# suleka96/siddhi

Hardware: AMD Instinct MI355X
Metric: input events/sec + % HBM peak, partitioned pattern query, 1/2/4/8 MI355X (higher is better)
Workload: dtype f64

## Files before the change

### siddhi_amd/csrc/kernels/fastpath.h

```cpp
#pragma once
#include "nfa.h"
#include "primitives.h"
#include "stream_ops.h"

namespace sm {

struct FastArgs {
  int64_t n;
  const int64_t* ts;
  const NfaStream* st;
  const KeyProg* key;
  const Instr* code;
  const DVal* consts;
  int c1_off, c1_len, c2_off, c2_len;
  int64_t within;
  const int64_t* ordinals;
  int64_t ordinal_base;
};

struct FastHostInfo {
  const void* const* cols;
  const int32_t* types;
  int key_col = -1;
  int key_type = 0;
// ... 43 lines not shown
    ts_last = 0;
  }
};

int64_t fast_every_within(const FastArgs& a, uint32_t* pairs_out, int64_t pairs_cap, Scratch& sc, hipStream_t s,
                          FastTimings* tm = nullptr);

enum : int64_t { FAST_OUTSIDE = -1, FAST_NON_MONOTONE = -2, FAST_KEY_SPAN = -3 };

int64_t fast_every_within_v2(const FastArgs& a, const FastHostInfo& hi, FastState& fs, FastCarry& carry,
                             uint32_t* pairs_out, int64_t pairs_cap, Scratch& sc, hipStream_t s,
                             FastTimings* tm = nullptr, int stack_mode = 0);

int64_t fast_seq_adjacent(const FastArgs& a, const FastHostInfo& hi, FastState& fs, FastCarry& carry,
                          uint32_t* pairs_out, int64_t pairs_cap, Scratch& sc, hipStream_t s, FastTimings* tm = nullptr);


struct StackPlan {
  const void* rec;
  const uint32_t* dbase;
  int64_t n;
  int64_t omax;
  int H;
  int64_t kmin;
  int op;
  bool fp;
  bool exact_codes;
  int vtype, vattr, vmode;
  int64_t vmin;
  const void* vcol;
  int64_t within;
  int64_t ts0, ts_last;
  int32_t o0;
};

int64_t stack_pipeline(const StackPlan& p, const FastArgs& a, const FastHostInfo& hi, FastState& fs, FastCarry& carry,
                       uint32_t* pairs_out, int64_t pairs_cap, Scratch& sc, hipStream_t s, FastTimings* tm);

void build_carry(const int64_t* cand, int64_t ncand, const NfaStream* st, int nattr, FastCarry& carry, Scratch& sc,
                 hipStream_t s, int key_bits = 64, int64_t kmin = 0, bool key_runs_ordered = false);

void pair_project(const uint32_t* pairs, int64_t m, const NfaStream* st_dev, const int64_t* ord, int64_t n,
                  int64_t base, const int64_t* ts, const int64_t* prev_carry, int64_t nc, int cw, const char* blob_dev,
                  DVal* out, int64_t* ts_out, Scratch& sc, hipStream_t s, bool rows = false,
                  int64_t* words = nullptr, uint8_t* nulls = nullptr,
                  const uint32_t* carry_keys = nullptr, const uint32_t* carry_idx = nullptr, bool sync = true);
void pair_project_carry_order(const int64_t* prev_carry, int64_t nc, int cw, int64_t base, Scratch& sc, hipStream_t s,
                              const uint32_t** carry_keys, const uint32_t** carry_idx);

}
```

### siddhi_amd/csrc/kernels/fastpath3.hip

```cpp
#include <cstdlib>
#include <type_traits>
#include <vector>

#include "expr.h"
#include "fastpath.h"
#include "fastpath_dev.h"
#include "pass0_dev.h"

#ifndef SM_ORIG_NT_LOAD
#define SM_ORIG_NT_LOAD 1
#endif

namespace sm {

namespace {

#ifndef SM_SB
#define SM_SB 512
#endif
#ifndef SM_SI
#define SM_SI 8
#endif
constexpr int kBlock = SM_SB;
constexpr int kWaves = kBlock / 64;
constexpr int kItems = SM_SI;
constexpr int kTile = kBlock * kItems;
constexpr int kBinsPerThread = kBins >= kBlock ? kBins / kBlock : 1;
constexpr int kUpUnroll = 8;
#ifndef SM_WB
#define SM_WB 512
#endif
#ifndef SM_WI
#define SM_WI 4
// ... 141 lines not shown
    unsigned long long e = __shfl_down(vlo, o, 64), f = __shfl_down(vhi, o, 64);
    lo = x < lo ? x : lo;
    hi = y > hi ? y : hi;
    om = z > om ? z : om;
    vlo = e < vlo ? e : vlo;
    vhi = f > vhi ? f : vhi;
  }
  bad = __any(bad) ? 1u : 0u;
  bado = __any(bado) ? 1u : 0u;
  if (lane == 0) {
    if (kcol) {
      atomicMin(&c->kmin, lo);
      atomicMax(&c->kmax, hi);
    }
    if (vlong) {
      atomicMin(&c->vmin, vlo);
      atomicMax(&c->vmax, vhi);
    }
    if (ord) atomicMax(&c->omax, om);
    if (bad) atomicOr(&c->bad_ts, 1u);
    if (bado) atomicOr(&c->bad_ord, 1u);
  }
  if (blockIdx.x == 0 && threadIdx.x == 0) {
    c->ts0 = ts[0];
    c->ts_last = ts[n - 1];
    c->o0 = ord ? ord[0] - obase : 0;
    if (!ord) c->omax = (unsigned long long)(n - 1);
  }
  __syncthreads();
  if (kcol)
    for (int d = threadIdx.x; d < kBins; d += kBlock) cnt[(int64_t)d * G + blockIdx.x] = h[d];
}


template <typename KT>
struct KeyColDigits {
  const KT* kcol;
  int64_t kmin;
  __device__ uint32_t key(int64_t p) const { return (uint32_t)((int64_t)kcol[p] - kmin); }
};
struct RecDigits {
  const uint4* r;
  __device__ uint32_t key(int64_t p) const { return ((const uint32_t*)r)[4 * p]; }
};
struct PairDigits {
  const uint64_t* q;
  __device__ uint32_t key(int64_t p) const { return (uint32_t)(q[p] >> 32); }
};

template <typename DS>
__global__ void __launch_bounds__(kBlock) upsweep_kernel(DS src, int64_t n, int64_t per, int G, int shift,
                                                         uint32_t* __restrict__ cnt) {
  __shared__ uint32_t h[kBins];
  for (int d = threadIdx.x; d < kBins; d += kBlock) h[d] = 0;
  __syncthreads();
  int64_t lo, len;
  chunk_range(blockIdx.x, n, per, nullptr, lo, len);
  const int64_t hi = lo + len;
  for (int64_t b = lo; b < hi; b += (int64_t)kBlock * kUpUnroll) {
    uint32_t k[kUpUnroll];
#pragma unroll
    for (int u = 0; u < kUpUnroll; ++u) {
      const int64_t p = b + u * kBlock + threadIdx.x;
      k[u] = p < hi ? src.key(p) : 0u;
    }
#pragma unroll
// ... 33 lines not shown
  uint32_t v[kBinsPerThread], s = 0;
  for (int k = 0; k < kBinsPerThread; ++k) {
    const int d = threadIdx.x * kBinsPerThread + k;
    v[k] = d < kBins ? tot[d] : 0u;
    s += v[k];
  }
  const int lane = threadIdx.x & 63, w = threadIdx.x >> 6;
  const uint32_t inc = wave_incl_scan(s);
  if (lane == 63) lw[w] = inc;
  __syncthreads();
  uint32_t run = inc - s;
  for (int k = 0; k < w; ++k) run += lw[k];
  for (int k = 0; k < kBinsPerThread; ++k) {
    if (threadIdx.x * kBinsPerThread + k < kBins) tot[threadIdx.x * kBinsPerThread + k] = run;
    run += v[k];
  }
}


template <typename VT>
struct ValLoader {
  VT v;
  __device__ StackVal var(const Instr&) const {
    StackVal r;
    r.i = 0;
    r.d = 0;
    r.null = 0;
    if constexpr (std::is_floating_point<VT>::value) r.d = (double)v;
    else r.i = (int64_t)v;
    return r;
  }
};

template <typename KT, typename VT>
struct OrigSrc {
  const NfaStream* st;
  const KT* kcol;
  const VT* vcol;
  int64_t kmin;
  int vmode;
  int64_t vmin;
  const uint64_t* c1mask;
  const int64_t* ts;
  int64_t ts0;
  const int64_t* ord;
  int64_t obase;
  const Instr* c1code;
  int c1len;
  const DVal* consts;
  bool c1_inline;
  Cond c1;
  __device__ void init() {
    if (c1_inline) c1 = make_cond(c1code, c1len, consts);
  }
  __device__ uint32_t c1_bit(VT v, uint64_t m, int64_t p) const {
    if (c1_inline) return eval_simple(c1, ValLoader<VT>{v}) ? 1u : 0u;
    return (uint32_t)(m >> (p & 63)) & 1u;
  }
  __device__ uint4 rec(int64_t p) const {
    uint4 r;
    const VT v = vcol[p];
    const uint64_t m = c1_inline ? 0ull : c1mask[p >> 6];
    r.x = (uint32_t)((int64_t)kcol[p] - kmin) | (c1_bit(v, m, p) << 31);
    r.y = ord ? (uint32_t)(ord[p] - obase) : (uint32_t)p;
    r.z = vcode<VT>(v, vmode, vmin);
    r.w = (uint32_t)(ts[p] - ts0);
    return r;
  }
  struct Raw {
    uint32_t k;
    VT v;
    uint32_t t, o, m;
  };
  __device__ Raw load(int64_t p) const {
    Raw r;
    const uint32_t* t32 = (const uint32_t*)(ts + p);
#if SM_ORIG_NT_LOAD
    r.k = __builtin_nontemporal_load((const uint32_t*)(kcol + p));
    r.v = __builtin_nontemporal_load(vcol + p);
    r.t = __builtin_nontemporal_load(t32);
    if (ord) r.o = __builtin_nontemporal_load((const uint32_t*)(ord + p));
#else
    r.k = *(const uint32_t*)(kcol + p);
    r.v = vcol[p];
    r.t = *t32;
    if (ord) r.o = *(const uint32_t*)(ord + p);
#endif
    if (!c1_inline) r.m = ((const uint32_t*)c1mask)[p >> 5];
    return r;
  }
  __device__ uint32_t rel_ord(const Raw& r, int64_t p) const { return ord ? r.o - (uint32_t)obase : (uint32_t)p; }
  __device__ uint32_t c1_of(const Raw& r, int64_t p) const {
    if (c1_inline) return eval_simple(c1, ValLoader<VT>{r.v}) ? 1u : 0u;
    return (r.m >> (p & 31)) & 1u;
  }
  __device__ void split(const Raw& r, int64_t p, uint64_t& a, uint64_t& b) const {
    const uint32_t c1 = c1_of(r, p);
    a = (uint64_t)((r.k - (uint32_t)kmin) | (c1 << 31)) | ((uint64_t)rel_ord(r, p) << 32);
    b = (uint64_t)vcode<VT>(r.v, vmode, vmin) | ((uint64_t)(r.t - (uint32_t)ts0) << 32);
  }
  __device__ uint4 record(const Raw& r, int64_t p) const {
    const uint32_t c1 = c1_of(r, p);
    return make_uint4((r.k - (uint32_t)kmin) | (c1 << 31), rel_ord(r, p), vcode<VT>(r.v, vmode, vmin),
                      r.t - (uint32_t)ts0);
  }
  __device__ void flush() {}
};

struct RecSrc {
  const uint4* r;
  __device__ void init() {}
  typedef unsigned int Raw __attribute__((ext_vector_type(4)));
  __device__ uint4 rec(int64_t p) const {
    const Raw v = __builtin_nontemporal_load((const Raw*)r + p);
    return make_uint4(v.x, v.y, v.z, v.w);
  }
  __device__ Raw load(int64_t p) const { return __builtin_nontemporal_load((const Raw*)r + p); }
  __device__ void split(const Raw& v, int64_t, uint64_t& a, uint64_t& b) const {
    a = (uint64_t)v.x | ((uint64_t)v.y << 32);
    b = (uint64_t)v.z | ((uint64_t)v.w << 32);
  }
};

struct PairSrc {
  const uint64_t* q;
  __device__ void init() {}
  using Raw = uint64_t;
  __device__ Raw load(int64_t p) const { return __builtin_nontemporal_load(q + p); }
  __device__ void split(const Raw& v, int64_t, uint64_t& a, uint64_t&) const { a = v; }
};

template <int MODE, typename Src>
__global__ void __launch_bounds__(kBlock) __attribute__((amdgpu_waves_per_eu(4)))
downsweep_kernel(Src src, uint4* __restrict__ drec, uint64_t* __restrict__ dpairs, int64_t n, int64_t per,
                 const uint32_t* seg_len, int G, int shift, const uint32_t* __restrict__ cnt,
                 const uint32_t* __restrict__ dbase) {
  __shared__ uint64_t xb64[kTile];
// ... 972 lines not shown

bool sort_wc() {
  static const bool on = [] {
    const char* e = getenv("SM_SORT_WC");
    return !(e && e[0] == '0');
  }();
  return on;
}

int jpass_wc() {
  static const int v = [] {
    const char* e = getenv("SM_JPASS_WC");
    return e ? atoi(e) : 0;
  }();
  return v;
}

bool c1_inline(const FastHostInfo& hi, const FastArgs& a) {
  if (!hi.c1_host || hi.c1_len != a.c1_len) return false;
  if (hi.c1_len != 0) {
    const Instr* c = hi.c1_host;
    auto leaf = [](const Instr& in) { return in.op != OP_CMP && in.op != OP_MATH && in.op != OP_NOT; };
    if (hi.c1_len != 3 || c[2].op != OP_CMP || !leaf(c[0]) || !leaf(c[1])) return false;
  }
  for (int k = 0; k < hi.c1_len; ++k) {
    const Instr& in = hi.c1_host[k];
    if (in.op == OP_TS) return false;
    if (in.op == OP_VAR && (in.a != 0 || in.c != hi.vattr)) return false;
    if (in.op == OP_COL && in.a != hi.vattr) return false;
  }
  return true;
}

template <typename KT, typename VT>
void launch_down0_t(const FastHostInfo& hi, const FastArgs& a, const void* kcol, int64_t kmin, int vmode, int64_t vmin,
                    const uint64_t* c1mask, int64_t ts0, int G, int64_t per, hipStream_t s, uint4* dst,
                    const uint32_t* cnt, const uint32_t* dbase) {
  OrigSrc<KT, VT> os{a.st, (const KT*)kcol, (const VT*)hi.cols[hi.vattr], kmin, vmode, vmin, c1mask, a.ts, ts0,
                     a.ordinals, a.ordinal_base, a.code + a.c1_off, a.c1_len, a.consts, c1_inline(hi, a)};
  static const bool p0v2 = !(getenv("SM_PASS0_V2") && getenv("SM_PASS0_V2")[0] == '0');
  if (sort_wc() && p0v2)
    hipLaunchKernelGGL((pass0_kernel<OrigSrc<KT, VT>>), dim3(G), dim3(kP0Block), 0, s, os, dst, a.n, per, G, cnt, dbase);
  else if (sort_wc())
    hipLaunchKernelGGL((downsweep_wc_kernel<0, OrigSrc<KT, VT>>), dim3(G), dim3(kWcBlock), 0, s, os, dst, nullptr, a.n,
                       per, nullptr, G, 0, cnt, dbase);
  else
    hipLaunchKernelGGL((downsweep_kernel<0, OrigSrc<KT, VT>>), dim3(G), dim3(kBlock), 0, s, os, dst, nullptr, a.n, per,
                       nullptr, G, 0, cnt, dbase);
}

template <typename KT>
void launch_down0_k(const FastHostInfo& hi, const FastArgs& a, const void* kcol, int64_t kmin, int vmode, int64_t vmin,
                    const uint64_t* m, int64_t ts0, int G, int64_t per, hipStream_t s, uint4* dst,
                    const uint32_t* cnt, const uint32_t* dbase) {
  switch (hi.vtype) {
    case T_INT: launch_down0_t<KT, int32_t>(hi, a, kcol, kmin, vmode, vmin, m, ts0, G, per, s, dst, cnt, dbase); break;
    case T_LONG: launch_down0_t<KT, int64_t>(hi, a, kcol, kmin, vmode, vmin, m, ts0, G, per, s, dst, cnt, dbase); break;
    case T_FLOAT: launch_down0_t<KT, float>(hi, a, kcol, kmin, vmode, vmin, m, ts0, G, per, s, dst, cnt, dbase); break;
    case T_DOUBLE: launch_down0_t<KT, double>(hi, a, kcol, kmin, vmode, vmin, m, ts0, G, per, s, dst, cnt, dbase); break;
    default: throw std::runtime_error("fast path: unsupported compared-attribute type");
  }
}

int64_t round_up(int64_t x, int64_t m) { return (x + m - 1) / m * m; }


struct ResolveArgs {
  const int64_t* crow;
  int64_t nc;
  int w, vattr, vtype, vmode;
  int64_t vmin;
  bool exact_codes;
  const uint4* rec;
  const NfaStream* st;
  const int64_t* ts;
  const int64_t* ord;
  int64_t obase, n, kmin, span, ts0, within;
  uint64_t* cpair;
  int64_t* cand;
  uint32_t* cand_n;
  uint32_t cand_cap;
  uint32_t* err;
};

template <bool KEYED, int OP, bool FP>
__global__ void resolve_kernel(ResolveArgs r) {
  const int64_t i = (int64_t)blockIdx.x * blockDim.x + threadIdx.x;
  if (i >= r.nc) return;
  const int64_t* row = r.crow + i * r.w;
  const int64_t key = row[0], oc = row[1], tc = row[2];
  const StackVal vc = uncanon((uint64_t)row[3 + r.vattr], r.vtype);
  r.cpair[i] = ~0ull;
// ... 183 lines not shown

  if (fs.cus == 0) {
    int dev = 0;
    SM_HIP(hipGetDevice(&dev));
    SM_HIP(hipDeviceGetAttribute(&fs.cus, hipDeviceAttributeMultiprocessorCount, dev));
  }
  if (fs.sort_wgs_per_cu == 0) {
    int b = 0;
    if (sort_wc()) SM_HIP(hipOccupancyMaxActiveBlocksPerMultiprocessor(&b, downsweep_wc_kernel<1, RecSrc>, kWcBlock, 0));
    else SM_HIP(hipOccupancyMaxActiveBlocksPerMultiprocessor(&b, downsweep_kernel<1, RecSrc>, kBlock, 0));
    fs.sort_wgs_per_cu = std::max(1, b);
    b = 0;
    SM_HIP(hipOccupancyMaxActiveBlocksPerMultiprocessor(&b, walk_kernel<true, CMP_GT, true>, kWalkBlock, 0));
    fs.walk_wgs_per_cu = std::max(1, b);
  }
  constexpr int kOversub = 2;
  const int64_t tiles = (n + kTile - 1) / kTile;
  const int G = (int)std::max<int64_t>(1, std::min<int64_t>(tiles, (int64_t)kOversub * fs.sort_wgs_per_cu * fs.cus));
  const int64_t per = round_up((n + G - 1) / G, kTile);
  const int64_t wtiles = (n + kWalkTile - 1) / kWalkTile;
  const int Gw = (int)std::max<int64_t>(1, std::min<int64_t>(wtiles, (int64_t)fs.walk_wgs_per_cu * fs.cus));
  const int64_t perw = round_up((n + Gw - 1) / Gw, kWalkTile);
  uint32_t* cnt = (uint32_t*)sc.take(sizeof(uint32_t) * kBins * std::max(G, Gw));
  uint32_t* dbase = (uint32_t*)sc.take(sizeof(uint32_t) * kBins);
  uint32_t* mcount = (uint32_t*)sc.take(sizeof(uint32_t) * Gw);
  uint64_t* c1mask = (uint64_t*)sc.take(((n + 63) / 64) * 8);
  auto scan_counts = [&](int g) {
    hipLaunchKernelGGL(scan_chunks_kernel, dim3(kBins), dim3(256), 0, s, cnt, g, dbase);
    hipLaunchKernelGGL(digit_base_kernel, dim3(1), dim3(kBlock), 0, s, dbase);
    tmark("scan");
  };

  const bool mask = !keyed || !c1_inline(hi, a);
#define SM_PREP2(KT, M, X)                                                                                          \
  hipLaunchKernelGGL((prep_kernel<KT, M, X>), dim3(G), dim3(kBlock), 0, s, (const KT*)kcol, vlong, a.ts, a.ordinals, \
                     a.ordinal_base, n, per, G, a.st, a.code + a.c1_off, a.c1_len, a.consts, c1mask, cnt, c)
#define SM_PREP(KT, M)                  \
  do {                                  \
    if (a.ordinals || vlong)            \
      SM_PREP2(KT, M, true);            \
    else                                \
      SM_PREP2(KT, M, false);           \
  } while (0)
  if (key_type == T_LONG && keyed) {
    if (mask) SM_PREP(int64_t, true);
    else SM_PREP(int64_t, false);
  } else {
    if (mask) SM_PREP(int32_t, true);
    else SM_PREP(int32_t, false);
  }
#undef SM_PREP
#undef SM_PREP2
  tmark("prep");
  Ctrl hc;
  SM_HIP(hipMemcpyAsync(&hc, c, sizeof(Ctrl), hipMemcpyDeviceToHost, s));
  SM_HIP(hipStreamSynchronize(s));
  if (a.within >= 0) {
    if (hc.bad_ts || (carry.active && hc.ts0 < carry.ts_last)) {
      sc.used = mark;
      return FAST_NON_MONOTONE;
    }
    if ((unsigned long long)(hc.ts_last - hc.ts0) >= 0xffffffffull) return bail();
  }
  if (hc.omax >= 0x7fffffffull || hc.bad_ord) return bail();
  int kbits = 0;
  int64_t kmin = 0;
  uint64_t kspan = 0;
  if (keyed) {
    kmin = (int64_t)(hc.kmin ^ 0x8000000000000000ull);
    kmin &= ~(int64_t)(kBins - 1);
    kspan = (uint64_t)((int64_t)(hc.kmax ^ 0x8000000000000000ull) - kmin);
    kbits = std::max(1, bits_for(kspan));
    if (kbits > 30 || (hi.remap_span > 0 && kspan > (uint64_t)hi.remap_span)) {
      sc.used = mark;
      return FAST_KEY_SPAN;
    }
  }
  int vmode = VC_I32;
  int64_t vmin = 0;
  bool exact_codes = true;
  switch (hi.vtype) {
    case T_INT: vmode = VC_I32; break;
    case T_FLOAT: vmode = VC_F32; break;
    case T_DOUBLE: vmode = VC_F64; exact_codes = false; break;
    default:
      if (keyed && carry.n == 0 && hc.vmax - hc.vmin <= 0xffffffffull) {
        vmode = VC_I64R;
        vmin = (int64_t)(hc.vmin ^ 0x8000000000000000ull);
      } else {
        vmode = VC_I64H;
        exact_codes = false;
      }
  }
  const int fpass = keyed ? (kbits + kRB - 1) / kRB : 0;
  const int jbits = std::max(1, bits_for(hc.omax));
  const int jpass = (jbits + kRB - 1) / kRB;
  auto finish = [&](int64_t m) {
    carry.ts_last = carry.active ? std::max<int64_t>(carry.ts_last, hc.ts_last) : (int64_t)hc.ts_last;
    carry.active = true;
    sc.used = mark;
    return m;
  };

  uint64_t* stq = nullptr;
  uint64_t *pq = nullptr, *qq = nullptr;
  WalkArgs wa{};
  wa.st = a.st;
  wa.ts = a.ts;
  wa.ord = a.ordinals;
  wa.obase = a.ordinal_base;
  wa.c1 = a.code + a.c1_off;
  wa.c1_len = a.c1_len;
  wa.c2 = a.code + a.c2_off;
  wa.c2_len = a.c2_len;
  wa.consts = a.consts;
  wa.vattr = hi.vattr;
  wa.vtype = hi.vtype;
  wa.within = a.within;
  wa.n = n;
  wa.exact_codes = exact_codes;
  wa.c1mask = c1mask;
  wa.kmin = kmin;
  wa.ts0 = hc.ts0;
  const int64_t nc = carry.n;
  const int64_t cand_cap = std::min<int64_t>(n + nc, (int64_t)1 << 26) + 1024;
  uint32_t* cflags = (uint32_t*)sc.take(16);
  SM_HIP(hipMemsetAsync(cflags, 0, 16, s));
  int64_t* cand = nullptr;
  uint4* cur = nullptr;
  if (keyed) {
    uint4* A = (uint4*)sc.take(n * 16);
    uint4* B = (uint4*)sc.take(n * 16);
    scan_counts(G);
    if (key_type == T_INT)
      launch_down0_k<int32_t>(hi, a, kcol, kmin, vmode, vmin, c1mask, hc.ts0, G, per, s, A, cnt, dbase);
    else launch_down0_k<int64_t>(hi, a, kcol, kmin, vmode, vmin, c1mask, hc.ts0, G, per, s, A, cnt, dbase);
    tmark("key_pass0");
    const int H = (int)std::min<uint64_t>(kspan >> kRB, 1ull << 20) + 1;
    const bool order_op = spec >= 0 && (spec >> 1) != CMP_EQ && (spec >> 1) != CMP_NE;
    const bool ts_ok = a.within < 0 || (a.within < (1ll << 30) && hc.ts_last - hc.ts0 < (1ll << 30));
    if (stack_mode != 2 && order_op && ts_ok && H <= kBins && (stack_mode == 1 || H >= kBins / 2)) {
      StackPlan sp{};
      sp.rec = A;
      sp.dbase = dbase;
      sp.n = n;
      sp.omax = (int64_t)hc.omax;
      sp.H = H;
      sp.kmin = kmin;
      sp.op = spec >> 1;
      sp.fp = (spec & 1) != 0;
      sp.exact_codes = exact_codes;
      sp.vtype = hi.vtype;
      sp.vattr = hi.vattr;
      sp.vmode = vmode;
      sp.vmin = vmin;
      sp.vcol = hi.cols[hi.vattr];
      sp.within = a.within;
      sp.ts0 = hc.ts0;
      sp.ts_last = hc.ts_last;
      sp.o0 = (int32_t)hc.o0;
      const int64_t m = stack_pipeline(sp, a, hi, fs, carry, pairs_out, pairs_cap, sc, s, tm);
      if (m >= 0) {
        fs.last_path = 3;
        if (tm) {
          SM_HIP(hipEventRecord(tm->ev[1], s));
          SM_HIP(hipEventRecord(tm->ev[2], s));
          SM_HIP(hipEventRecord(tm->ev[3], s));
        }
        return finish(m);
      }
    }
    cand = (int64_t*)sc.take((size_t)cand_cap * 32);
    cur = A;
    uint4* nxt = B;
    for (int p = 1; p < fpass; ++p) {
      hipLaunchKernelGGL((upsweep_kernel<RecDigits>), dim3(G), dim3(kBlock), 0, s, RecDigits{cur}, n, per, G,
                         p * kRB, cnt);
      tmark("key_up");
      scan_counts(G);
      if (sort_wc())
        hipLaunchKernelGGL((downsweep_wc_kernel<1, RecSrc>), dim3(G), dim3(kWcBlock), 0, s, RecSrc{cur}, nxt, nullptr, n,
                           per, nullptr, G, p * kRB, cnt, dbase);
      else
        hipLaunchKernelGGL((downsweep_kernel<1, RecSrc>), dim3(G), dim3(kBlock), 0, s, RecSrc{cur}, nxt, nullptr, n,
                           per, nullptr, G, p * kRB, cnt, dbase);
      tmark("key_pass");
      std::swap(cur, nxt);
    }
    if (tm) SM_HIP(hipEventRecord(tm->ev[1], s));
    wa.rec = cur;
    wa.cand = cand;
    wa.cand_n = cflags;
    wa.cand_cap = (uint32_t)cand_cap;
    wa.err = cflags + 1;
// ... 162 lines not shown
```

### siddhi_amd/csrc/kernels/pass0_dev.h

```cpp
#pragma once
#include "fastpath_dev.h"

namespace sm {
namespace {

constexpr int kP0Block = 1024;
constexpr int kP0Waves = kP0Block / 64;
constexpr int kP0Items = 4;
constexpr int kP0Tile = kP0Block * kP0Items;
constexpr int kP0Seg = 4;
static_assert(kBins == kP0Block && kP0Waves == 16, "one digit per thread, 16 waves");

__device__ __forceinline__ uint32_t sm_udot2(uint32_t a, uint32_t b, uint32_t c) {
#if defined(__HIP_DEVICE_COMPILE__)
  typedef unsigned short u16x2 __attribute__((ext_vector_type(2)));
  return __builtin_amdgcn_udot2(__builtin_bit_cast(u16x2, a), __builtin_bit_cast(u16x2, b), c, false);
#else
  return c + (a & 0xffffu) * (b & 0xffffu) + (a >> 16) * (b >> 16);
#endif
}

__device__ __forceinline__ uint32_t p0_before(const uint4& r0, const uint4& r1, int w) {
  const uint32_t word[8] = {r0.x, r0.y, r0.z, r0.w, r1.x, r1.y, r1.z, r1.w};
  uint32_t s = 0;
#pragma unroll
  for (int i = 0; i < 8; ++i) {
    const uint32_t m = 2 * i + 1 < w ? 0xffffffffu : (2 * i < w ? 0x0000ffffu : 0u);
    s = sm_udot2(word[i] & m, 0x00010001u, s);
  }
  return s;
}

__device__ __forceinline__ void p0_store_fence(uint4 (&rec)[kP0Items]) {
#if defined(__HIP_DEVICE_COMPILE__)
#pragma unroll
  for (int k = 0; k < kP0Items; ++k)
    asm volatile("" : "+v"(rec[k].x), "+v"(rec[k].y), "+v"(rec[k].z), "+v"(rec[k].w) : : "memory");
#else
  (void)rec;
#endif
}

__device__ __forceinline__ int64_t p0_opaque(int64_t v) {
#if defined(__HIP_DEVICE_COMPILE__)
  asm volatile("" : "+s"(v));
#endif
  return v;
}

template <typename Src>
__global__ void __launch_bounds__(kP0Block) pass0_kernel(Src src, uint4* __restrict__ drec, int64_t n, int64_t per,
                                                          int G, const uint32_t* __restrict__ cnt,
                                                          const uint32_t* __restrict__ dbase) {
  __shared__ __attribute__((aligned(16))) uint4 xb[kP0Tile];
  __shared__ __attribute__((aligned(16))) uint16_t wc[kBins][kP0Waves];
  __shared__ uint32_t tstart[kBins + 1];
  __shared__ uint32_t run[kBins];
  __shared__ uint32_t cst[kBins];
  __shared__ __attribute__((aligned(16))) uint4 carry[kBins][kP0Seg - 1];
  __shared__ uint32_t lw[kP0Waves];

  const int tid = threadIdx.x, lane = tid & 63, w = wave_index();
  const int64_t lo = (int64_t)blockIdx.x * per;
  int64_t len = n - lo;
  if (len > per) len = per;
  if (len < 0) len = 0;
  src.init();
  uint4* row = (uint4*)&wc[tid][0];
  {
    const uint32_t r0 = dbase[tid] + cnt[(int64_t)tid * G + blockIdx.x];
    run[tid] = r0;
    cst[tid] = r0;
    row[0] = make_uint4(0, 0, 0, 0);
    row[1] = make_uint4(0, 0, 0, 0);
  }
  lds_barrier();
  typename Src::Raw raw[kP0Items];
  auto load_tile = [&](int64_t base) {
    const int64_t rem = lo + len - base;
    const int tn = rem < kP0Tile ? (int)rem : kP0Tile;
    base = p0_opaque(base);
#pragma unroll
    for (int k = 0; k < kP0Items; ++k) {
      const int e = w * 64 * kP0Items + k * 64 + lane;
      if (e < tn) raw[k] = src.load(base + e);
    }
  };
  const int64_t end = lo + len;
  if (len > 0) load_tile(lo);
  int ptile_n = 0;
  bool plast = false;
  uint4 cq0, cq1, cq2;
  static_assert(kP0Seg == 4, "three carried records at most");

  for (int64_t base = lo;; base += kP0Tile) {
    const bool more = base < end;
    const int tile_n = (int)((end - base) < kP0Tile ? (end - base) : kP0Tile);
    const bool last = base + kP0Tile >= end;
    uint4 rec[kP0Items];
#if defined(__HIP_DEVICE_COMPILE__)
    __builtin_amdgcn_s_waitcnt(0x0F70);
#endif
    if (more) {
#pragma unroll
      for (int k = 0; k < kP0Items; ++k) {
        const int e = w * 64 * kP0Items + k * 64 + lane;
        if (e < tile_n) rec[k] = src.record(raw[k], base + e);
      }
    }
    p0_store_fence(rec);

    if (base != lo) {
      const uint32_t rn = run[tid], c0 = cst[tid], ct = tstart[tid + 1] - tstart[tid];
      const uint32_t lim = plast ? 0xffffffffu : ((rn + ct) & ~(uint32_t)(kP0Seg - 1));
      const uint32_t nfl = (rn != c0 && (plast || lim > c0)) ? rn - c0 : 0u;
      if (nfl > 0) drec[c0] = cq0;
      if (nfl > 1) drec[c0 + 1] = cq1;
      if (nfl > 2) drec[c0 + 2] = cq2;
#pragma unroll
      for (int r = 0; r < kP0Items; ++r) {
        const int s = r * kP0Block + tid;
        if (s < ptile_n) {
          const uint4 x = xb[s];
          const uint32_t d = x.x & (kBins - 1);
          const uint32_t rd = run[d], td = tstart[d];
          const uint32_t dest = rd + (uint32_t)s - td;
          const uint32_t ld = plast ? 0xffffffffu : ((rd + tstart[d + 1] - td) & ~(uint32_t)(kP0Seg - 1));
          if (dest < ld) {
            drec[dest] = x;
          } else {
            const uint32_t cd = cst[d];
            carry[d][dest - (cd > ld ? cd : ld)] = x;
          }
        }
      }
      lds_barrier();
      run[tid] = rn + ct;
      if (lim != 0xffffffffu && lim > c0) cst[tid] = lim;
    }
    if (!more) break;

    uint32_t dg[kP0Items], lp = 0;
    static_assert(kP0Items * 64 <= 256 && kP0Items <= 4, "a record's rank within (wave, digit) fits 8 bits");
#pragma unroll
    for (int k = 0; k < kP0Items; ++k) {
      const int e = w * 64 * kP0Items + k * 64 + lane;
      const bool valid = e < tile_n;
      dg[k] = valid ? rec[k].x & (kBins - 1) : 0u;
      const uint64_t peers = peer_mask(dg[k], valid);
      uint32_t old = 0;
      if (valid) old = wc[dg[k]][w];
      wave_lockstep();
      const uint32_t below = lanes_below(peers);
      if (valid && below == 0) wc[dg[k]][w] = (uint16_t)(old + (uint32_t)__popcll(peers));
      wave_lockstep();
      lp |= (old + below) << (8 * k);
    }
    if (!last) load_tile(base + kP0Tile);
    lds_barrier();

    uint32_t ct = 0;
    {
      const uint4 r0 = row[0], r1 = row[1];
      const uint32_t word[8] = {r0.x, r0.y, r0.z, r0.w, r1.x, r1.y, r1.z, r1.w};
#pragma unroll
      for (int i = 0; i < 8; ++i) ct = sm_udot2(word[i], 0x00010001u, ct);
      uint32_t tot;
      tstart[tid] = block_excl<kP0Block>(ct, lw, &tot);
      if (tid == 0) tstart[kBins] = tot;
    }
    const uint32_t rn = run[tid], c0 = cst[tid];
    const uint32_t lim = last ? 0xffffffffu : ((rn + ct) & ~(uint32_t)(kP0Seg - 1));
    lds_barrier();

#pragma unroll
    for (int k = 0; k < kP0Items; ++k) {
      const int e = w * 64 * kP0Items + k * 64 + lane;
      if (e < tile_n) {
        const uint32_t d = rec[k].x & (kBins - 1);
        const uint4* rr = (const uint4*)&wc[d][0];
        xb[tstart[d] + p0_before(rr[0], rr[1], w) + ((lp >> (8 * k)) & 0xffu)] = rec[k];
      }
    }
    const uint32_t nfl = (rn != c0 && (last || lim > c0)) ? rn - c0 : 0u;
    if (nfl > 0) cq0 = carry[tid][0];
    if (nfl > 1) cq1 = carry[tid][1];
    if (nfl > 2) cq2 = carry[tid][2];
    lds_barrier();
    row[0] = make_uint4(0, 0, 0, 0);
    row[1] = make_uint4(0, 0, 0, 0);
    ptile_n = tile_n;
    plast = last;
  }
  src.flush();
}

}
}
```

### siddhi_amd/csrc/kernels/stack.hip

```cpp
#include <cstdio>
#include <cstdlib>
#include <vector>

#include "fastpath.h"
#include "stack_dev.h"
#include "order_dev.h"

namespace sm {

namespace {

#ifndef SM_STACK_KPT
#define SM_STACK_KPT 2
#endif
constexpr int kKPT = SM_STACK_KPT;
constexpr int kSB = kKeys / kKPT;
constexpr int kSW = kSB / 64;
#ifndef SM_STACK_KSI
#define SM_STACK_KSI (SM_STACK_KPT == 2 ? 9 : 4)
#endif
constexpr int kSI = SM_STACK_KSI;
constexpr int kS = kSB * kSI;
constexpr int kLog = 4096;
constexpr int kOvf = 1024;
// ... 674 lines not shown
  uint64_t* kord = (uint64_t*)sc.take((size_t)ncand * 8);
  uint64_t* kkey = (uint64_t*)sc.take((size_t)ncand * 8);
  uint64_t* k2 = (uint64_t*)sc.take((size_t)ncand * 8);
  uint32_t* idx = (uint32_t*)sc.take((size_t)ncand * 4);
  uint32_t* idx2 = (uint32_t*)sc.take((size_t)ncand * 4);
  hipLaunchKernelGGL(carry_rows_kernel, grid_of(ncand), dim3(256), 0, s, cand, ncand, st, nattr,
                     (const int64_t*)carry.rows, w, kmin, key_bits, rows, kord, kkey, idx);
  const uint32_t* fin;
  if (key_runs_ordered) {
    const bool alt = radix_sort_pairs<uint64_t>(kkey, k2, idx, idx2, (size_t)ncand, 0, key_bits, sc, s);
    fin = alt ? idx2 : idx;
  } else {
    bool alt = radix_sort_pairs<uint64_t>(kord, k2, idx, idx2, (size_t)ncand, 0, 64, sc, s);
    uint32_t* i1 = alt ? idx2 : idx;
    uint32_t* i1b = alt ? idx : idx2;
    hipLaunchKernelGGL(gather_u64_kernel, grid_of(ncand), dim3(256), 0, s, kkey, i1, ncand, k2);
    alt = radix_sort_pairs<uint64_t>(k2, kkey, i1, i1b, (size_t)ncand, 0, key_bits, sc, s);
    fin = alt ? i1b : i1;
  }
  carry.reserve(ncand, w);
  hipLaunchKernelGGL(gather_rows_kernel, grid_of(ncand), dim3(256), 0, s, rows, fin, ncand, w, carry.rows);
  SM_HIP(hipStreamSynchronize(s));
  carry.n = ncand;
  sc.used = mark;
}

int64_t stack_pipeline(const StackPlan& p, const FastArgs& a, const FastHostInfo& hi, FastState& fs, FastCarry& carry,
                       uint32_t* pairs_out, int64_t pairs_cap, Scratch& sc, hipStream_t s, FastTimings* tm) {
  const size_t mark = sc.used;
  auto tmark = [&](const char* l) {
    if (tm) tm->mark(l, s);
  };
  const int64_t n = p.n;
  uint32_t* err = (uint32_t*)sc.take(16);
  uint32_t* cand_n = err + 1;
  uint32_t* stot = err + 2;
  SM_HIP(hipMemsetAsync(err, 0, 16, s));
  StackArgs sa{};
  sa.rec = (const uint4*)p.rec;
  sa.dbase = p.dbase;
  sa.ntiles = (p.omax >> kTB) + 1;
  sa.n = n;
  sa.H = p.H;
  sa.kmin = p.kmin;
  sa.within = p.within;
  sa.ts0 = p.ts0;
  sa.exact_codes = p.exact_codes;
  sa.vtype = p.vtype;
  sa.vcol = p.vcol;
  sa.ord = a.ordinals;
  sa.obase = a.ordinal_base;
  sa.o0 = p.o0;
  sa.vattr = p.vattr;
  sa.err = err;

  int64_t nc = carry.n;
  const int64_t cand_cap = std::min<int64_t>(n + nc, (int64_t)8 * p.H * kBins + nc) + 1024;
  sa.cand = (int64_t*)sc.take((size_t)cand_cap * 32);
  sa.cand_n = cand_n;
  sa.cand_cap = (uint32_t)std::min<int64_t>(cand_cap, 0xffffffffll);
  uint32_t* ccnt = nullptr;
  if (nc > 0) {
    const int64_t span = (int64_t)p.H << kRB;
    uint4* cin = (uint4*)sc.take((size_t)nc * 16);
    uint32_t* cst = (uint32_t*)sc.take((size_t)span * 4);
    uint32_t* cen = (uint32_t*)sc.take((size_t)span * 4);
    ccnt = (uint32_t*)sc.take(kBins * 4);
    SM_HIP(hipMemsetAsync(cst, 0, (size_t)span * 4, s));
    SM_HIP(hipMemsetAsync(cen, 0, (size_t)span * 4, s));
    SM_HIP(hipMemsetAsync(ccnt, 0, kBins * 4, s));
#define SM_CIN(VT)                                                                                                  \
  hipLaunchKernelGGL((carry_in_kernel<VT>), grid_of(nc), dim3(256), 0, s, (const int64_t*)carry.rows, nc, carry.width, \
                     p.vattr, p.vtype, p.vmode, p.vmin, p.kmin, span - 1, a.ordinal_base, p.o0, p.ts0, cin, cst, cen, ccnt,  \
                     sa.cand, cand_n, err)
    switch (p.vtype) {
      case T_INT: SM_CIN(int32_t); break;
      case T_LONG: SM_CIN(int64_t); break;
      case T_FLOAT: SM_CIN(float); break;
      default: SM_CIN(double); break;
    }
#undef SM_CIN
    sa.cin = cin;
    sa.cstart = cst;
    sa.cend = cen;
    sa.crow = (const int64_t*)carry.rows;
    sa.cwidth = carry.width;
  }
  uint32_t* sbase = (uint32_t*)sc.take(kBins * 4);
  hipLaunchKernelGGL(stage_base_kernel, dim3(1), dim3(kOB), 0, s, p.dbase, ccnt, sbase, stot);
  uint32_t hs[3];
  SM_HIP(hipMemcpyAsync(hs, err, 12, hipMemcpyDeviceToHost, s));
  SM_HIP(hipStreamSynchronize(s));
  if (hs[0] & SE_ORD) {
    sc.used = mark;
    throw std::runtime_error("a carried partial lies more than 2^31 events before the batch's ordinal base (match "
                             "tuples are 32-bit ordinals relative to it), or not before the batch");
  }
  const int64_t extra = hs[2];
  const int64_t ncand_in = hs[1];
  if (fs.cus == 0) {
    int dev = 0;
    SM_HIP(hipGetDevice(&dev));
    SM_HIP(hipDeviceGetAttribute(&fs.cus, hipDeviceAttributeMultiprocessorCount, dev));
  }
  static const bool v2 = getenv("SM_STACK_V2") && atoi(getenv("SM_STACK_V2")) != 0;
  int64_t M = 0;
  {
    sa.sbase = sbase;
    sa.stage = (uint64_t*)sc.take((size_t)(n + extra) * 8);
    sa.mstart = (uint32_t*)sc.take((size_t)kBins * (sa.ntiles + 1) * 4);
    sa.mtot = (uint32_t*)sc.take(kBins * 4);
    if (fs.cus == 0) {
      int dev = 0;
      SM_HIP(hipGetDevice(&dev));
      SM_HIP(hipDeviceGetAttribute(&fs.cus, hipDeviceAttributeMultiprocessorCount, dev));
    }
    const int grid = std::min(kBins, fs.cus);
    sa.spill = (uint4*)sc.take((size_t)grid * kKeys * kQ * 16);
    static const bool want_stamps = getenv("SM_STACK_STAMPS") != nullptr;
    static const int dbg = getenv("SM_STACK_DEBUG") ? atoi(getenv("SM_STACK_DEBUG")) : 0;
    sa.dbg = dbg;
    if (want_stamps) {
      sa.stamps = (unsigned long long*)sc.take(128);
      sa.counts = sa.stamps + 8;
      SM_HIP(hipMemsetAsync(sa.stamps, 0, 128, s));
// ... 268 lines not shown
```

Measured before the change: 28.31 billion.

## Defer timestamp monotonicity check from prep pass into pass 0 kernel

Adds a lighter prep_keys_kernel that reads only the key column (min/max plus histogram) and skips the timestamp order scan when keys are present, c1 is inline and there is no ordinal column. The timestamp order check moves into pass0_kernel, which already loads the full 64-bit timestamps. It compares neighbouring lanes via DPP and across waves and tiles through shared memory, and reports a flag that the stack pipeline or the host reads back. The aim is to drop one full read of the timestamp column in the prep pass. The cost is more complex control flow and extra fallback kernels on the bail paths.

New measurement: 29.60 billion, median of 6. 4.5% higher.

```diff
diff --git a/siddhi_amd/csrc/kernels/fastpath.h b/siddhi_amd/csrc/kernels/fastpath.h
--- a/siddhi_amd/csrc/kernels/fastpath.h
+++ b/siddhi_amd/csrc/kernels/fastpath.h
@@ -99,6 +99,7 @@
   int64_t within;
   int64_t ts0, ts_last;
   int32_t o0;
+  uint32_t* status = nullptr;
 };
 
 int64_t stack_pipeline(const StackPlan& p, const FastArgs& a, const FastHostInfo& hi, FastState& fs, FastCarry& carry,
diff --git a/siddhi_amd/csrc/kernels/fastpath3.hip b/siddhi_amd/csrc/kernels/fastpath3.hip
--- a/siddhi_amd/csrc/kernels/fastpath3.hip
+++ b/siddhi_amd/csrc/kernels/fastpath3.hip
@@ -1,4 +1,5 @@
 #include <cstdlib>
+#include <limits>
 #include <type_traits>
 #include <vector>
 
@@ -206,6 +207,65 @@
     for (int d = threadIdx.x; d < kBins; d += kBlock) cnt[(int64_t)d * G + blockIdx.x] = h[d];
 }
 
+constexpr int kKeyItems = 16;
+template <typename KT>
+__global__ void __launch_bounds__(kBlock) prep_keys_kernel(const KT* __restrict__ kcol, const int64_t* __restrict__ ts,
+                                                           int64_t n, int64_t per, int G, uint32_t* __restrict__ cnt,
+                                                           Ctrl* __restrict__ c) {
+  __shared__ uint32_t h[kBins];
+  for (int d = threadIdx.x; d < kBins; d += kBlock) h[d] = 0;
+  __syncthreads();
+  int64_t lo0, len;
+  chunk_range(blockIdx.x, n, per, nullptr, lo0, len);
+  const int64_t hi0 = lo0 + len;
+  KT kmn = std::numeric_limits<KT>::max(), kmx = std::numeric_limits<KT>::min();
+  for (int64_t base = lo0; base < hi0; base += (int64_t)kBlock * kKeyItems) {
+    KT kk[kKeyItems];
+#pragma unroll
+    for (int k = 0; k < kKeyItems; ++k) {
+      const int64_t p = base + k * kBlock + threadIdx.x;
+      if (p < hi0) kk[k] = __builtin_nontemporal_load(kcol + p);
+    }
+#pragma unroll
+    for (int k = 0; k < kKeyItems; ++k) {
+      const int64_t p = base + k * kBlock + threadIdx.x;
+      if (p < hi0) {
+        kmn = kmn < kk[k] ? kmn : kk[k];
+        kmx = kmx > kk[k] ? kmx : kk[k];
+        atomicAdd(&h[(uint32_t)kk[k] & (kBins - 1)], 1u);
+      }
+    }
+  }
+  const bool any = lo0 + (int64_t)threadIdx.x < hi0;
+  unsigned long long lo = any ? (unsigned long long)(int64_t)kmn ^ 0x8000000000000000ull : ~0ull;
+  unsigned long long hi = any ? (unsigned long long)(int64_t)kmx ^ 0x8000000000000000ull : 0ull;
+  for (int o = 32; o > 0; o >>= 1) {
+    const unsigned long long x = __shfl_down(lo, o, 64), y = __shfl_down(hi, o, 64);
+    lo = x < lo ? x : lo;
+    hi = y > hi ? y : hi;
+  }
+  if ((threadIdx.x & 63) == 0) {
+    atomicMin(&c->kmin, lo);
+    atomicMax(&c->kmax, hi);
+  }
+  if (blockIdx.x == 0 && threadIdx.x == 0) {
+    c->ts0 = ts[0];
+    c->ts_last = ts[n - 1];
+    c->o0 = 0;
+    c->omax = (unsigned long long)(n - 1);
+  }
+  __syncthreads();
+  for (int d = threadIdx.x; d < kBins; d += kBlock) cnt[(int64_t)d * G + blockIdx.x] = h[d];
+}
+
+__global__ void __launch_bounds__(256) ts_order_kernel(const int64_t* __restrict__ ts, int64_t n,
+                                                       Ctrl* __restrict__ c) {
+  bool bad = false;
+  for (int64_t p = (int64_t)blockIdx.x * 256 + threadIdx.x + 1; p < n; p += (int64_t)gridDim.x * 256)
+    bad |= ts[p] < ts[p - 1];
+  if (bad) atomicOr(&c->bad_ts, 1u);
+}
+
 
 template <typename KT>
 struct KeyColDigits {
@@ -305,7 +365,7 @@
   }
 };
 
-template <typename KT, typename VT>
+template <typename KT, typename VT, bool TS = false>
 struct OrigSrc {
   const NfaStream* st;
   const KT* kcol;
@@ -322,20 +382,27 @@
   int c1len;
   const DVal* consts;
   bool c1_inline;
+  uint32_t* ts_flag;
   Cond c1;
+  static constexpr bool kTimeOrder = TS;
+  __device__ bool has_ord() const { return !TS && ord != nullptr; }
+  __device__ bool inl() const { return TS || c1_inline; }
+  __device__ int64_t time0() const { return ts0; }
+  __device__ int64_t time_at(int64_t p) const { return ts[p]; }
+  __device__ void time_bad() const { atomicOr(ts_flag, 1u); }
   __device__ void init() {
-    if (c1_inline) c1 = make_cond(c1code, c1len, consts);
+    if (inl()) c1 = make_cond(c1code, c1len, consts);
   }
   __device__ uint32_t c1_bit(VT v, uint64_t m, int64_t p) const {
-    if (c1_inline) return eval_simple(c1, ValLoader<VT>{v}) ? 1u : 0u;
+    if (inl()) return eval_simple(c1, ValLoader<VT>{v}) ? 1u : 0u;
     return (uint32_t)(m >> (p & 63)) & 1u;
   }
   __device__ uint4 rec(int64_t p) const {
     uint4 r;
     const VT v = vcol[p];
-    const uint64_t m = c1_inline ? 0ull : c1mask[p >> 6];
+    const uint64_t m = inl() ? 0ull : c1mask[p >> 6];
     r.x = (uint32_t)((int64_t)kcol[p] - kmin) | (c1_bit(v, m, p) << 31);
-    r.y = ord ? (uint32_t)(ord[p] - obase) : (uint32_t)p;
+    r.y = has_ord() ? (uint32_t)(ord[p] - obase) : (uint32_t)p;
     r.z = vcode<VT>(v, vmode, vmin);
     r.w = (uint32_t)(ts[p] - ts0);
     return r;
@@ -343,39 +410,42 @@
   struct Raw {
     uint32_t k;
     VT v;
-    uint32_t t, o, m;
+    typename std::conditional<TS, int64_t, uint32_t>::type t;
+    uint32_t o, m;
   };
+  __device__ int64_t time_of(const Raw& r) const { return (int64_t)r.t; }
   __device__ Raw load(int64_t p) const {
     Raw r;
-    const uint32_t* t32 = (const uint32_t*)(ts + p);
+    typedef typename std::conditional<TS, int64_t, uint32_t>::type TT;
+    const TT* t32 = (const TT*)(ts + p);
 #if SM_ORIG_NT_LOAD
     r.k = __builtin_nontemporal_load((const uint32_t*)(kcol + p));
     r.v = __builtin_nontemporal_load(vcol + p);
     r.t = __builtin_nontemporal_load(t32);
-    if (ord) r.o = __builtin_nontemporal_load((const uint32_t*)(ord + p));
+    if (has_ord()) r.o = __builtin_nontemporal_load((const uint32_t*)(ord + p));
 #else
     r.k = *(const uint32_t*)(kcol + p);
     r.v = vcol[p];
     r.t = *t32;
-    if (ord) r.o = *(const uint32_t*)(ord + p);
+    if (has_ord()) r.o = *(const uint32_t*)(ord + p);
 #endif
-    if (!c1_inline) r.m = ((const uint32_t*)c1mask)[p >> 5];
+    if (!inl()) r.m = ((const uint32_t*)c1mask)[p >> 5];
     return r;
   }
-  __device__ uint32_t rel_ord(const Raw& r, int64_t p) const { return ord ? r.o - (uint32_t)obase : (uint32_t)p; }
+  __device__ uint32_t rel_ord(const Raw& r, int64_t p) const { return has_ord() ? r.o - (uint32_t)obase : (uint32_t)p; }
   __device__ uint32_t c1_of(const Raw& r, int64_t p) const {
-    if (c1_inline) return eval_simple(c1, ValLoader<VT>{r.v}) ? 1u : 0u;
+    if (inl()) return eval_simple(c1, ValLoader<VT>{r.v}) ? 1u : 0u;
     return (r.m >> (p & 31)) & 1u;
   }
   __device__ void split(const Raw& r, int64_t p, uint64_t& a, uint64_t& b) const {
     const uint32_t c1 = c1_of(r, p);
     a = (uint64_t)((r.k - (uint32_t)kmin) | (c1 << 31)) | ((uint64_t)rel_ord(r, p) << 32);
-    b = (uint64_t)vcode<VT>(r.v, vmode, vmin) | ((uint64_t)(r.t - (uint32_t)ts0) << 32);
+    b = (uint64_t)vcode<VT>(r.v, vmode, vmin) | ((uint64_t)((uint32_t)r.t - (uint32_t)ts0) << 32);
   }
   __device__ uint4 record(const Raw& r, int64_t p) const {
     const uint32_t c1 = c1_of(r, p);
     return make_uint4((r.k - (uint32_t)kmin) | (c1 << 31), rel_ord(r, p), vcode<VT>(r.v, vmode, vmin),
-                      r.t - (uint32_t)ts0);
+                      (uint32_t)r.t - (uint32_t)ts0);
   }
   __device__ void flush() {}
 };
@@ -1414,14 +1484,31 @@
   return true;
 }
 
+bool pass0_v2() {
+  static const bool on = !(getenv("SM_PASS0_V2") && getenv("SM_PASS0_V2")[0] == '0');
+  return sort_wc() && on;
+}
+
 template <typename KT, typename VT>
 void launch_down0_t(const FastHostInfo& hi, const FastArgs& a, const void* kcol, int64_t kmin, int vmode, int64_t vmin,
                     const uint64_t* c1mask, int64_t ts0, int G, int64_t per, hipStream_t s, uint4* dst,
-                    const uint32_t* cnt, const uint32_t* dbase) {
+                    const uint32_t* cnt, const uint32_t* dbase, uint32_t* ts_flag) {
+  if (ts_flag) {
+    if constexpr (std::is_same<VT, int64_t>::value) {
+      throw std::logic_error("the time-order check of pass 0 is not built for a LONG compared attribute");
+    } else {
+      if (!pass0_v2() || a.ordinals || !c1_inline(hi, a))
+        throw std::logic_error("the time-order check of pass 0: pass0_kernel, no ordinal column, c1 inline");
+      OrigSrc<KT, VT, true> os{a.st, (const KT*)kcol, (const VT*)hi.cols[hi.vattr], kmin, vmode, vmin, c1mask, a.ts,
+                               ts0, a.ordinals, a.ordinal_base, a.code + a.c1_off, a.c1_len, a.consts, true, ts_flag};
+      hipLaunchKernelGGL((pass0_kernel<OrigSrc<KT, VT, true>>), dim3(G), dim3(kP0Block), 0, s, os, dst, a.n, per, G,
+                         cnt, dbase);
+    }
+    return;
+  }
   OrigSrc<KT, VT> os{a.st, (const KT*)kcol, (const VT*)hi.cols[hi.vattr], kmin, vmode, vmin, c1mask, a.ts, ts0,
-                     a.ordinals, a.ordinal_base, a.code + a.c1_off, a.c1_len, a.consts, c1_inline(hi, a)};
-  static const bool p0v2 = !(getenv("SM_PASS0_V2") && getenv("SM_PASS0_V2")[0] == '0');
-  if (sort_wc() && p0v2)
+                     a.ordinals, a.ordinal_base, a.code + a.c1_off, a.c1_len, a.consts, c1_inline(hi, a), nullptr};
+  if (pass0_v2())
     hipLaunchKernelGGL((pass0_kernel<OrigSrc<KT, VT>>), dim3(G), dim3(kP0Block), 0, s, os, dst, a.n, per, G, cnt, dbase);
   else if (sort_wc())
     hipLaunchKernelGGL((downsweep_wc_kernel<0, OrigSrc<KT, VT>>), dim3(G), dim3(kWcBlock), 0, s, os, dst, nullptr, a.n,
@@ -1434,12 +1521,16 @@
 template <typename KT>
 void launch_down0_k(const FastHostInfo& hi, const FastArgs& a, const void* kcol, int64_t kmin, int vmode, int64_t vmin,
                     const uint64_t* m, int64_t ts0, int G, int64_t per, hipStream_t s, uint4* dst,
-                    const uint32_t* cnt, const uint32_t* dbase) {
+                    const uint32_t* cnt, const uint32_t* dbase, uint32_t* tf) {
   switch (hi.vtype) {
-    case T_INT: launch_down0_t<KT, int32_t>(hi, a, kcol, kmin, vmode, vmin, m, ts0, G, per, s, dst, cnt, dbase); break;
-    case T_LONG: launch_down0_t<KT, int64_t>(hi, a, kcol, kmin, vmode, vmin, m, ts0, G, per, s, dst, cnt, dbase); break;
-    case T_FLOAT: launch_down0_t<KT, float>(hi, a, kcol, kmin, vmode, vmin, m, ts0, G, per, s, dst, cnt, dbase); break;
-    case T_DOUBLE: launch_down0_t<KT, double>(hi, a, kcol, kmin, vmode, vmin, m, ts0, G, per, s, dst, cnt, dbase); break;
+    case T_INT: launch_down0_t<KT, int32_t>(hi, a, kcol, kmin, vmode, vmin, m, ts0, G, per, s, dst, cnt, dbase, tf);
+      break;
+    case T_LONG: launch_down0_t<KT, int64_t>(hi, a, kcol, kmin, vmode, vmin, m, ts0, G, per, s, dst, cnt, dbase, tf);
+      break;
+    case T_FLOAT: launch_down0_t<KT, float>(hi, a, kcol, kmin, vmode, vmin, m, ts0, G, per, s, dst, cnt, dbase, tf);
+      break;
+    case T_DOUBLE: launch_down0_t<KT, double>(hi, a, kcol, kmin, vmode, vmin, m, ts0, G, per, s, dst, cnt, dbase, tf);
+      break;
     default: throw std::runtime_error("fast path: unsupported compared-attribute type");
   }
 }
@@ -1689,6 +1780,7 @@
   };
 
   const bool mask = !keyed || !c1_inline(hi, a);
+  const bool late_ts = keyed && !mask && !a.ordinals && !vlong && pass0_v2();
 #define SM_PREP2(KT, M, X)                                                                                          \
   hipLaunchKernelGGL((prep_kernel<KT, M, X>), dim3(G), dim3(kBlock), 0, s, (const KT*)kcol, vlong, a.ts, a.ordinals, \
                      a.ordinal_base, n, per, G, a.st, a.code + a.c1_off, a.c1_len, a.consts, c1mask, cnt, c)
@@ -1699,7 +1791,14 @@
     else                                \
       SM_PREP2(KT, M, false);           \
   } while (0)
-  if (key_type == T_LONG && keyed) {
+  if (late_ts) {
+    if (key_type == T_LONG)
+      hipLaunchKernelGGL((prep_keys_kernel<int64_t>), dim3(G), dim3(kBlock), 0, s, (const int64_t*)kcol, a.ts, n, per, G,
+                         cnt, c);
+    else
+      hipLaunchKernelGGL((prep_keys_kernel<int32_t>), dim3(G), dim3(kBlock), 0, s, (const int32_t*)kcol, a.ts, n, per, G,
+                         cnt, c);
+  } else if (key_type == T_LONG && keyed) {
     if (mask) SM_PREP(int64_t, true);
     else SM_PREP(int64_t, false);
   } else {
@@ -1712,12 +1811,27 @@
   Ctrl hc;
   SM_HIP(hipMemcpyAsync(&hc, c, sizeof(Ctrl), hipMemcpyDeviceToHost, s));
   SM_HIP(hipStreamSynchronize(s));
+  auto late_bad_ts = [&]() -> bool {
+    if (!late_ts || a.within < 0) return false;
+    hipLaunchKernelGGL(ts_order_kernel, dim3((unsigned)std::min<int64_t>((n + 255) / 256, 4096)), dim3(256), 0, s, a.ts,
+                       n, c);
+    unsigned int bad = 0;
+    SM_HIP(hipMemcpyAsync(&bad, &c->bad_ts, sizeof bad, hipMemcpyDeviceToHost, s));
+    SM_HIP(hipStreamSynchronize(s));
+    return bad != 0;
+  };
   if (a.within >= 0) {
     if (hc.bad_ts || (carry.active && hc.ts0 < carry.ts_last)) {
       sc.used = mark;
       return FAST_NON_MONOTONE;
     }
-    if ((unsigned long long)(hc.ts_last - hc.ts0) >= 0xffffffffull) return bail();
+    if ((unsigned long long)(hc.ts_last - hc.ts0) >= 0xffffffffull) {
+      if (late_bad_ts()) {
+        sc.used = mark;
+        return FAST_NON_MONOTONE;
+      }
+      return bail();
+    }
   }
   if (hc.omax >= 0x7fffffffull || hc.bad_ord) return bail();
   int kbits = 0;
@@ -1729,8 +1843,9 @@
     kspan = (uint64_t)((int64_t)(hc.kmax ^ 0x8000000000000000ull) - kmin);
     kbits = std::max(1, bits_for(kspan));
     if (kbits > 30 || (hi.remap_span > 0 && kspan > (uint64_t)hi.remap_span)) {
+      const bool bad = late_bad_ts();
       sc.used = mark;
-      return FAST_KEY_SPAN;
+      return bad ? FAST_NON_MONOTONE : FAST_KEY_SPAN;
     }
   }
   int vmode = VC_I32;
@@ -1788,15 +1903,31 @@
   if (keyed) {
     uint4* A = (uint4*)sc.take(n * 16);
     uint4* B = (uint4*)sc.take(n * 16);
-    scan_counts(G);
-    if (key_type == T_INT)
-      launch_down0_k<int32_t>(hi, a, kcol, kmin, vmode, vmin, c1mask, hc.ts0, G, per, s, A, cnt, dbase);
-    else launch_down0_k<int64_t>(hi, a, kcol, kmin, vmode, vmin, c1mask, hc.ts0, G, per, s, A, cnt, dbase);
-    tmark("key_pass0");
     const int H = (int)std::min<uint64_t>(kspan >> kRB, 1ull << 20) + 1;
     const bool order_op = spec >= 0 && (spec >> 1) != CMP_EQ && (spec >> 1) != CMP_NE;
     const bool ts_ok = a.within < 0 || (a.within < (1ll << 30) && hc.ts_last - hc.ts0 < (1ll << 30));
-    if (stack_mode != 2 && order_op && ts_ok && H <= kBins && (stack_mode == 1 || H >= kBins / 2)) {
+    const bool stack = stack_mode != 2 && order_op && ts_ok && H <= kBins && (stack_mode == 1 || H >= kBins / 2);
+    uint32_t* sstat = nullptr;
+    if (late_ts && stack) {
+      sstat = (uint32_t*)sc.take(16);
+      SM_HIP(hipMemsetAsync(sstat, 0, 16, s));
+    }
+    uint32_t* ts_flag = late_ts ? (stack ? sstat + 3 : cflags + 2) : nullptr;
+    scan_counts(G);
+    if (key_type == T_INT)
+      launch_down0_k<int32_t>(hi, a, kcol, kmin, vmode, vmin, c1mask, hc.ts0, G, per, s, A, cnt, dbase, ts_flag);
+    else launch_down0_k<int64_t>(hi, a, kcol, kmin, vmode, vmin, c1mask, hc.ts0, G, per, s, A, cnt, dbase, ts_flag);
+    tmark("key_pass0");
+    if (late_ts && !stack && a.within >= 0) {
+      uint32_t bad = 0;
+      SM_HIP(hipMemcpyAsync(&bad, ts_flag, 4, hipMemcpyDeviceToHost, s));
+      SM_HIP(hipStreamSynchronize(s));
+      if (bad) {
+        sc.used = mark;
+        return FAST_NON_MONOTONE;
+      }
+    }
+    if (stack) {
       StackPlan sp{};
       sp.rec = A;
       sp.dbase = dbase;
@@ -1816,7 +1947,12 @@
       sp.ts0 = hc.ts0;
       sp.ts_last = hc.ts_last;
       sp.o0 = (int32_t)hc.o0;
+      sp.status = sstat;
       const int64_t m = stack_pipeline(sp, a, hi, fs, carry, pairs_out, pairs_cap, sc, s, tm);
+      if (m == FAST_NON_MONOTONE) {
+        sc.used = mark;
+        return FAST_NON_MONOTONE;
+      }
       if (m >= 0) {
         fs.last_path = 3;
         if (tm) {
diff --git a/siddhi_amd/csrc/kernels/pass0_dev.h b/siddhi_amd/csrc/kernels/pass0_dev.h
--- a/siddhi_amd/csrc/kernels/pass0_dev.h
+++ b/siddhi_amd/csrc/kernels/pass0_dev.h
@@ -1,4 +1,6 @@
 #pragma once
+#include <type_traits>
+
 #include "fastpath_dev.h"
 
 namespace sm {
@@ -46,6 +48,19 @@
   asm volatile("" : "+s"(v));
 #endif
   return v;
+}
+
+template <typename S, typename = void>
+struct p0_time_order : std::false_type {};
+template <typename S>
+struct p0_time_order<S, std::void_t<decltype(S::kTimeOrder)>> : std::integral_constant<bool, S::kTimeOrder> {};
+
+__device__ __forceinline__ uint32_t p0_lane_before(uint32_t v) {
+#if defined(__HIP_DEVICE_COMPILE__)
+  return (uint32_t)__builtin_amdgcn_update_dpp((int)v, (int)v, 0x138 , 0xf, 0xf, false);
+#else
+  return __shfl_up(v, 1, 64);
+#endif
 }
 
 template <typename Src>
@@ -59,6 +74,9 @@
   __shared__ uint32_t cst[kBins];
   __shared__ __attribute__((aligned(16))) uint4 carry[kBins][kP0Seg - 1];
   __shared__ uint32_t lw[kP0Waves];
+  __shared__ uint32_t tlast[kP0Waves + 1];
+  __shared__ uint32_t tbad;
+  constexpr bool kTO = p0_time_order<Src>::value;
 
   const int tid = threadIdx.x, lane = tid & 63, w = wave_index();
   const int64_t lo = (int64_t)blockIdx.x * per;
@@ -74,7 +92,14 @@
     row[0] = make_uint4(0, 0, 0, 0);
     row[1] = make_uint4(0, 0, 0, 0);
   }
+  if constexpr (kTO) {
+    if (tid == 0) {
+      tbad = 0u;
+      tlast[kP0Waves] = (lo > 0 && len > 0) ? (uint32_t)(src.time_at(lo - 1) - src.time0()) : 0u;
+    }
+  }
   lds_barrier();
+  int tpar = 0;
   typename Src::Raw raw[kP0Items];
   auto load_tile = [&](int64_t base) {
     const int64_t rem = lo + len - base;
@@ -101,11 +126,35 @@
 #if defined(__HIP_DEVICE_COMPILE__)
     __builtin_amdgcn_s_waitcnt(0x0F70);
 #endif
+    uint32_t tfirst = 0;
     if (more) {
+      uint32_t tq[kP0Items];
+      bool tb = false;
 #pragma unroll
       for (int k = 0; k < kP0Items; ++k) {
         const int e = w * 64 * kP0Items + k * 64 + lane;
-        if (e < tile_n) rec[k] = src.record(raw[k], base + e);
+        if constexpr (kTO) tq[k] = 0u;
+        if (e < tile_n) {
+          rec[k] = src.record(raw[k], base + e);
+          if constexpr (kTO) {
+            const int64_t rel = src.time_of(raw[k]) - src.time0();
+            tq[k] = (uint32_t)rel;
+            tb |= ((uint64_t)rel >> 32) != 0;
+          }
+        }
+      }
+      if constexpr (kTO) {
+#pragma unroll
+        for (int k = 0; k < kP0Items; ++k) {
+          const int e = w * 64 * kP0Items + k * 64 + lane;
+          uint32_t pv = p0_lane_before(tq[k]);
+          const uint32_t pl = wave_read_lane(tq[k > 0 ? k - 1 : 0], 63);
+          if (lane == 0) pv = k > 0 ? pl : tq[0];
+          tb |= e < tile_n && tq[k] < pv;
+        }
+        if (lane == 63) tlast[w < kP0Waves - 1 ? w : kP0Waves - 1 + tpar] = tq[kP0Items - 1];
+        if (tb) tbad = 1u;
+        tfirst = tq[0];
       }
     }
     p0_store_fence(rec);
@@ -158,6 +207,11 @@
     }
     if (!last) load_tile(base + kP0Tile);
     lds_barrier();
+    if constexpr (kTO) {
+      if (lane == 0 && w * 64 * kP0Items < tile_n && tfirst < tlast[w > 0 ? w - 1 : kP0Waves - 1 + (tpar ^ 1)])
+        tbad = 1u;
+      tpar ^= 1;
+    }
 
     uint32_t ct = 0;
     {
@@ -193,7 +247,10 @@
     plast = last;
   }
   src.flush();
-}
-
-}
-}
+  if constexpr (kTO) {
+    if (tid == 0 && tbad != 0u) src.time_bad();
+  }
+}
+
+}
+}
diff --git a/siddhi_amd/csrc/kernels/stack.hip b/siddhi_amd/csrc/kernels/stack.hip
--- a/siddhi_amd/csrc/kernels/stack.hip
+++ b/siddhi_amd/csrc/kernels/stack.hip
@@ -730,10 +730,10 @@
     if (tm) tm->mark(l, s);
   };
   const int64_t n = p.n;
-  uint32_t* err = (uint32_t*)sc.take(16);
+  uint32_t* err = p.status ? p.status : (uint32_t*)sc.take(16);
   uint32_t* cand_n = err + 1;
   uint32_t* stot = err + 2;
-  SM_HIP(hipMemsetAsync(err, 0, 16, s));
+  if (!p.status) SM_HIP(hipMemsetAsync(err, 0, 16, s));
   StackArgs sa{};
   sa.rec = (const uint4*)p.rec;
   sa.dbase = p.dbase;
@@ -786,9 +786,13 @@
   }
   uint32_t* sbase = (uint32_t*)sc.take(kBins * 4);
   hipLaunchKernelGGL(stage_base_kernel, dim3(1), dim3(kOB), 0, s, p.dbase, ccnt, sbase, stot);
-  uint32_t hs[3];
-  SM_HIP(hipMemcpyAsync(hs, err, 12, hipMemcpyDeviceToHost, s));
+  uint32_t hs[4];
+  SM_HIP(hipMemcpyAsync(hs, err, 16, hipMemcpyDeviceToHost, s));
   SM_HIP(hipStreamSynchronize(s));
+  if (p.status && p.within >= 0 && hs[3]) {
+    sc.used = mark;
+    return FAST_NON_MONOTONE;
+  }
   if (hs[0] & SE_ORD) {
     sc.used = mark;
     throw std::runtime_error("a carried partial lies more than 2^31 events before the batch's ordinal base (match "
```
